# drtconway/zotmer

Hardware: AMD Instinct MI355X
Metric: Gk-mers/sec kmerize k=25 on synthetic 150bp FASTQ; achieved HBM GB/s fraction (higher is better)
Workload: dtype u64

## Files before the change

### zotmer_amd/csrc/strand_blocks.hip

```cpp
#include "tile_group.hpp"

namespace zk {

constexpr int SB_ITEMS = 16, SB_GROUPS = 2048;
constexpr u32 SB_GROUP_MAX = 128;
typedef TileSortSmem<SB_ITEMS, SB_GROUPS, false> StrandSmem;
constexpr int SB_BLOCK_BITS = 18;

__global__ __launch_bounds__(256) void strand_mirror_kernel(const u64* __restrict__ in, const u64* __restrict__ cuts, const u64* __restrict__ incl,
                                                            const u64* __restrict__ nwords, u32 chunks, int pack, int K, u64* __restrict__ out_m,
                                                            MirrorHist mh, const u32* __restrict__ list, u64* cursor, u64 m_cap) {
    __shared__ u32 bins[4 * 512];
    __shared__ u64 placed;
    const bool hist = mh.passes > 0;
    if (hist) {
        for (int q = threadIdx.x; q < 4 * 512; q += blockDim.x) bins[q] = 0;
        __syncthreads();
    }
    const u64 maxc = (1ull << pack) - 1;
    for (u32 t = blockIdx.x; t < chunks; t += gridDim.x) {
        const u32 v = list ? list[t] : t;
        const u64 cnt = nwords[v];
        u64 dst0 = incl[v] - cnt;
        if (list) {
            if (threadIdx.x == 0) placed = atomicAdd(cursor, cnt);
            __syncthreads();
            dst0 = placed;
            __syncthreads();
            if (dst0 + cnt > m_cap) continue;
        }
        const u64* src = in + cuts[v];
        for (u64 i0 = threadIdx.x; i0 < cnt; i0 += 4ull * blockDim.x) {
            u64 w4[4];
#pragma unroll
            for (int q = 0; q < 4; q++) {
                const u64 i = i0 + (u64)q * blockDim.x;
                w4[q] = i < cnt ? src[i] : 0;
            }
#pragma unroll
            for (int q = 0; q < 4; q++) {
                const u64 i = i0 + (u64)q * blockDim.x;
                if (i >= cnt) break;
                const u64 mw = (revcomp(K, w4[q] >> pack) << pack) | (w4[q] & maxc);
                out_m[dst0 + i] = mw;
                if (hist) {
#pragma unroll
                    for (int p = 0; p < 4; p++)
                        if (p < mh.passes) atomicAdd(&bins[p * 512 + ((u32)(mw >> mh.shift[p]) & ((1u << mh.bits[p]) - 1u))], 1u);
                }
            }
        }
    }
    if (hist) {
        __syncthreads();
        for (int q = threadIdx.x; q < mh.passes * 512; q += blockDim.x)
            if (bins[q]) atomicAdd(&mh.raw[q], (u64)bins[q]);
    }
}

__global__ void strand_starts_kernel(const u64* __restrict__ m, u64 n, int shift, u64* __restrict__ start) {
    const u32 g = blockIdx.x * blockDim.x + threadIdx.x;
    if (g > (1u << SB_BLOCK_BITS)) return;
    u64 lo = 0, hi = n;
    if (g == (1u << SB_BLOCK_BITS)) lo = n;
    while (lo < hi) {
        const u64 mid = (lo + hi) >> 1;
        if ((m[mid] >> shift) < (u64)g) lo = mid + 1; else hi = mid;
    }
    start[g] = lo;
}

struct StrandArgs {
    const u64* cw;
    const u64* cuts; const u64* nwords; const u64* incl;
    const u64* m;
    const u64* mstart;
    u64* ok; u32* oc;
    int pack;
    int pshift;
    u32* n_declined;
    u32* declined;
};

__device__ __forceinline__ bool strand_crowded(const StrandSmem& sm, int tid) {
    static_assert(SB_GROUPS == 4 * TS_BLOCK, "four groups a thread");
    u32 big = 0;
#pragma unroll
    for (int q = 0; q < 4; q++) big |= sm.start[4 * tid + q + 1] - sm.start[4 * tid + q] > SB_GROUP_MAX ? 1u : 0u;
    return __syncthreads_or((int)big) != 0;
}

__device__ __forceinline__ void strand_write(const StrandSmem& sm, const TileMap& tm, u32 m, u64* ok, u32* oc, int pack, int tid) {
    const u64 maxc = (1ull << pack) - 1;
    constexpr int E = 2;
    for (u32 i0 = (u32)tid; i0 < m; i0 += E * TS_BLOCK) {
        u32 i[E], place[E];
        u64 mine[E];
#pragma unroll
        for (int e = 0; e < E; e++) i[e] = i0 + e * TS_BLOCK;
        tile_rank<E, false>(sm, tm, i, m, mine, place);
#pragma unroll
        for (int e = 0; e < E; e++) {
            if (i[e] >= m) break;
            ok[place[e]] = mine[e] >> pack;
            oc[place[e]] = (u32)(mine[e] & maxc);
        }
    }
}

__global__ __launch_bounds__(TS_BLOCK, 2 * TS_BLOCK / 256) void strand_block_union_kernel(StrandArgs a) {
    using S = StrandSmem;
    constexpr u32 CAP = S::CAP;
    static_assert(sizeof(S) <= 80 * 1024, "two workgroups per CU");
    __shared__ S sm;
    const u32 b = blockIdx.x;
    const u64 nc = a.nwords[b], m0 = a.mstart[b], nm = a.mstart[b + 1] - m0;
    const u64 n = nc + nm;
    if (n == 0) return;
    if (n > CAP) {
        if (threadIdx.x == 0) a.declined[atomicAdd(a.n_declined, 1u)] = b;
        return;
    }
    int tid = threadIdx.x;
    asm volatile("" : "+v"(tid));
    const u32 m = (u32)n;
    const TileMap tm = tile_group<SB_ITEMS, SB_GROUPS, false>(sm, a.cw, nullptr, a.cuts[b], m, a.pshift, tid, a.m, m0, (u32)nc);
    if (strand_crowded(sm, tid)) {
        if (tid == 0) a.declined[atomicAdd(a.n_declined, 1u)] = b;
        return;
    }
    const u64 out0 = a.incl[b] - nc + m0;
    strand_write(sm, tm, m, a.ok + out0, a.oc + out0, a.pack, tid);
}

constexpr int SB_SPLIT = 256;
struct StrandBigSmem {
    StrandSmem t;
    u64 sp[SB_SPLIT];
    u32 cnt[SB_SPLIT + 2];
    u32 tile[SB_SPLIT + 2];
    u32 ntiles, gcount, fail;
};

__global__ __launch_bounds__(TS_BLOCK) void strand_big_block_kernel(StrandArgs a, u32 n_list, u64* __restrict__ scratch, u32* __restrict__ fail) {
    using S = StrandBigSmem;
    constexpr u32 CAP = StrandSmem::CAP, R = SB_SPLIT + 1;
    __shared__ S sm;
    u64* gat = scratch + (u64)blockIdx.x * CAP;
    const int lane = threadIdx.x & 63;
    for (u32 li = blockIdx.x; li < n_list; li += gridDim.x) {
        int tid = threadIdx.x;
        asm volatile("" : "+v"(tid));
        const u32 b = a.declined[li];
        const u64 nc = a.nwords[b], m0 = a.mstart[b], nm = a.mstart[b + 1] - m0, n = nc + nm;
        const u64* C = a.cw + a.cuts[b];
        const u64* M = a.m + m0;
        auto entry = [&](u64 i) -> u64 { return i < nc ? C[i] : M[i - nc]; };
        const u64 bmin = (u64)b << a.pshift, bmax = bmin | ((1ull << a.pshift) - 1ull);
        const u64 out0 = a.incl[b] - nc + m0;
        u64* cand = sm.t.keys;
        if (tid < SB_SPLIT) cand[tid] = entry((u64)tid * n / SB_SPLIT);
        if (tid == 0) { sm.fail = 0; sm.gcount = 0; }
        if (tid < (int)R + 1) sm.cnt[tid] = 0;
        __syncthreads();
        if (tid < SB_SPLIT) {
            const u64 v = cand[tid];
            u32 r = 0;
            for (int q = 0; q < SB_SPLIT; q++) { const u64 o = cand[q]; r += (o < v || (o == v && q < tid)) ? 1u : 0u; }
            sm.sp[r] = v;
        }
        __syncthreads();
        auto range_of = [&](u64 v) -> u32 {
            u32 lo = 0, hi = SB_SPLIT;
            while (lo < hi) { const u32 mid = (lo + hi) >> 1; if (sm.sp[mid] <= v) lo = mid + 1; else hi = mid; }
            return lo;
        };
        for (u64 i = tid; i < n; i += TS_BLOCK) atomicAdd(&sm.cnt[range_of(entry(i))], 1u);
        __syncthreads();
        if (tid == 0) {
            u32 acc = 0, nt = 0, eb = 0;
            sm.tile[nt++] = 0;
            for (u32 j = 0; j < R; j++) {
                const u32 tot = sm.cnt[j];
                if (tot > CAP) { sm.fail = 1; break; }
                if (acc + tot > CAP) { sm.tile[nt++] = j; acc = 0; }
                acc += tot;
                sm.cnt[j] = eb;
                eb += tot;
            }
            sm.cnt[R] = eb;
            sm.tile[nt] = R;
            sm.ntiles = nt;
        }
        __syncthreads();
        if (sm.fail) {
            if (tid == 0) atomicOr(fail, 1u);
            continue;
        }
        const u32 ntiles = sm.ntiles;
        for (u32 t = 0; t < ntiles; t++) {
            const u32 ra = sm.tile[t], rb = sm.tile[t + 1];
            const u64 vlo = ra == 0 ? bmin : sm.sp[ra - 1];
            const u64 vhi = rb == R ? bmax : sm.sp[rb - 1] - 1;
            const u32 m = sm.cnt[rb] - sm.cnt[ra];
            if (m == 0) continue;
            for (u64 i0 = 0; i0 < n; i0 += TS_BLOCK) {
                const u64 i = i0 + tid;
                const u64 v = i < n ? entry(i) : 0;
                const bool in = i < n && v >= vlo && v <= vhi;
                const u64 bal = __ballot(in);
                u32 base = 0;
                if (lane == 0 && bal) base = atomicAdd(&sm.gcount, (u32)__popcll(bal));
                base = (u32)__shfl((int)base, 0, 64);
                if (in) gat[base + popc_below(bal)] = v;
            }
            __threadfence_block();
            __syncthreads();
            const TileMap tm = tile_group<SB_ITEMS, SB_GROUPS, false>(sm.t, gat, nullptr, 0, m, a.pshift, tid, nullptr, 0, ~0u, true, vlo, vhi);
            if (strand_crowded(sm.t, tid)) {
                if (tid == 0) atomicOr(fail, 1u);
                break;
            }
            const u64 o = out0 + sm.cnt[ra];
            strand_write(sm.t, tm, m, a.ok + o, a.oc + o, a.pack, tid);
            if (tid == 0) sm.gcount = 0;
            __syncthreads();
        }
        __syncthreads();
    }
}

constexpr int DS_ITEMS = 22, DS_GROUPS = 4096;
typedef TileSortSmem<DS_ITEMS, DS_GROUPS, false> BlockSortSmem;
static_assert(BlockSortSmem::CAP == 11264, "a dedupe2_kernel table");

__global__ __launch_bounds__(TS_BLOCK) void dedupe_sort_blocks_kernel(u64* __restrict__ w, const u64* __restrict__ cuts, const u64* __restrict__ nwords,
                                                                     u32 chunks, int pshift) {
    constexpr u32 CAP = BlockSortSmem::CAP;
    __shared__ BlockSortSmem sm;
    for (u32 v = blockIdx.x; v < chunks; v += gridDim.x) {
        const u64 n = nwords[v];
        if (n < 2 || n > CAP) continue;
        int tid = threadIdx.x;
        asm volatile("" : "+v"(tid));
        const u32 m = (u32)n;
        u64* out = w + cuts[v];
        const TileMap tm = tile_group<DS_ITEMS, DS_GROUPS, false>(sm, w, nullptr, cuts[v], m, pshift, tid);
        constexpr int E = 2;
        for (u32 i0 = (u32)tid; i0 < m; i0 += E * TS_BLOCK) {
            u32 i[E], place[E];
            u64 mine[E];
#pragma unroll
            for (int e = 0; e < E; e++) i[e] = i0 + e * TS_BLOCK;
            tile_rank<E, false>(sm, tm, i, m, mine, place);
#pragma unroll
            for (int e = 0; e < E; e++)
                if (i[e] < m) out[place[e]] = mine[e];
        }
        __syncthreads();
    }
}

int dedupe_sort_blocks(zk_ctx* c, DedupeResult& r) {
    if (!r.unsorted || r.n_out == 0) { r.unsorted = false; return ZK_OK; }
    prof_begin(c, ZK_PROF_RLE, 16 * r.n_out);
    hipLaunchKernelGGL(dedupe_sort_blocks_kernel, dim3(r.chunks < (u32)c->num_cus ? r.chunks : (u32)c->num_cus), dim3(TS_BLOCK), 0, c->stream, r.work, r.cuts,
                       r.nwords, r.chunks, r.tag_bits + r.pack);
    prof_end(c);
    ZK_HIP(c, hipGetLastError());
    r.unsorted = false;
    return ZK_OK;
}

int strand_blocks(zk_ctx* c, const DedupeResult& r, u64* keys_buf, uint64_t buf_words, int K, u64* out_k, u32* out_c, uint64_t cap,
                  uint64_t* n_out) {
    *n_out = 0;
    const uint64_t uc = r.n_out;
    if (uc == 0) return ZK_OK;
    if (!(K & 1) || r.n_big || r.chunks != (1u << SB_BLOCK_BITS)) return fail(c, ZK_EINTERNAL, "strand_blocks: K %d, %u big counts, %u blocks", K, r.n_big, r.chunks);
    const uint64_t a8w = ((8 * uc + 255) & ~255ull) / 8;
    if (2 * a8w > buf_words) return fail(c, ZK_EINTERNAL, "strand_blocks: %llu words do not fit twice in %llu", (unsigned long long)uc, (unsigned long long)buf_words);
    if (2 * uc > cap) return fail(c, ZK_ENOSPC, "output holds %llu entries, the table has %llu", (unsigned long long)cap, (unsigned long long)(2 * uc));
    const int pk = r.pack, key_bits = 2 * K + pk, lo_bit = key_bits - SB_BLOCK_BITS;
    u64* mw = keys_buf;
    u64* malt = keys_buf + a8w;
    MirrorHist mh = {};
    bool fused = r.m_emitted && r.m_words >= keys_buf && r.m_words + r.m_cap <= keys_buf + buf_words && uc <= r.m_cap && c->sort_variant == 3;
    if (fused) {
        const PassPlan plan = sort_plan_upper(c, key_bits, lo_bit);
        fused = plan.passes == r.mh.passes;
        for (int p = 0; fused && p < plan.passes; p++) fused = plan.shift[p] == r.mh.shift[p] && plan.bits[p] == r.mh.bits[p];
        const uint64_t before = (uint64_t)(r.m_words - keys_buf), behind = buf_words - before;
        if (before < a8w && behind < 2 * a8w) fused = false;
        if (fused) malt = before >= a8w ? keys_buf : r.m_words + a8w;
    }
    if (fused) {
        mw = r.m_words;
        mh = r.mh;
        uint64_t placed = r.m_placed;
        prof_begin(c, ZK_PROF_SELECT, 16 * uc);
        if (r.n_retry) {
            hipLaunchKernelGGL(strand_mirror_kernel, dim3(grid_cap(c, r.n_retry, 8)), dim3(256), 0, c->stream, r.work, r.cuts, r.incl, r.nwords, r.n_retry, pk, K,
                               mw, mh, r.retry, &c->d_scalars->dedupe_m_cursor, (u64)r.m_cap);
        }
        prof_end(c);
        if (r.n_retry) {
            ZK_HIP(c, hipGetLastError());
            ZK_TRY(fetch(c, &c->h_scalars->dedupe_m_cursor));
            ZK_TRY(stream_sync(c));
            placed = c->h_scalars->dedupe_m_cursor;
        }
        if (placed != uc) return fail(c, ZK_EINTERNAL, "strand_blocks: %llu mirror words for %llu entries", (unsigned long long)placed, (unsigned long long)uc);
    } else {
        if (c->sort_variant == 3) {
            const PassPlan plan = sort_plan_upper(c, key_bits, lo_bit);
            if (plan.passes <= 4) {
                ZK_TRY(arena_alloc(c, sizeof(u64) * MAX_PASSES * 512, (void**)&mh.raw));
                ZK_HIP(c, hipMemsetAsync(mh.raw, 0, sizeof(u64) * MAX_PASSES * 512, c->stream));
                mh.passes = plan.passes;
                for (int p = 0; p < plan.passes; p++) { mh.shift[p] = plan.shift[p]; mh.bits[p] = plan.bits[p]; }
            }
        }
        prof_begin(c, ZK_PROF_SELECT, 16 * uc);
        hipLaunchKernelGGL(strand_mirror_kernel, dim3((u32)c->num_cus * 8), dim3(256), 0, c->stream, r.work, r.cuts, r.incl, r.nwords, r.chunks, pk, K, mw, mh,
                           (const u32*)nullptr, (u64*)nullptr, (u64)0);
        prof_end(c);
        ZK_HIP(c, hipGetLastError());
    }
    u64* sk = nullptr;
    if (mh.passes) ZK_TRY(sort_keys_upper_counted(c, mw, malt, uc, key_bits, lo_bit, mh.raw, &sk));
    else ZK_TRY(sort_keys_upper(c, mw, malt, uc, key_bits, lo_bit, &sk));
    u64* mstart;
    u32* declined;
    ZK_TRY(arena_alloc(c, sizeof(u64) * ((1ull << SB_BLOCK_BITS) + 1), (void**)&mstart));
    ZK_TRY(arena_alloc(c, sizeof(u32) * r.chunks, (void**)&declined));
    StrandArgs a = {};
    a.cw = r.work; a.cuts = r.cuts; a.nwords = r.nwords; a.incl = r.incl; a.m = sk; a.mstart = mstart;
    a.ok = out_k; a.oc = out_c; a.pack = pk; a.pshift = lo_bit;
    a.n_declined = &c->d_scalars->strand.n_declined;
    a.declined = declined;
    u32* fail = &c->d_scalars->strand.fail;
    prof_begin(c, ZK_PROF_UNION, 8 * 2 * uc + 12 * 2 * uc);
    hipLaunchKernelGGL(strand_starts_kernel, dim3(((1u << SB_BLOCK_BITS) + 256) / 256), dim3(256), 0, c->stream, sk, (u64)uc, lo_bit, mstart);
    ZK_HIP(c, hipMemsetAsync(&c->d_scalars->strand, 0, sizeof(zk_strand_counters), c->stream));
    hipLaunchKernelGGL(strand_block_union_kernel, dim3(r.chunks), dim3(TS_BLOCK), 0, c->stream, a);
    prof_end(c);
    ZK_HIP(c, hipGetLastError());
    ZK_TRY(fetch(c, &c->h_scalars->strand));
    ZK_TRY(check_device_error(c));
    const uint32_t n_declined = c->h_scalars->strand.n_declined;
    bool other_way = n_declined && c->strand_blocks == 3;
    if (n_declined && !other_way) {
        const uint32_t grid = n_declined < 2u * (uint32_t)c->num_cus ? n_declined : 2u * (uint32_t)c->num_cus;
        u64* scratch;
        ZK_TRY(arena_alloc(c, sizeof(u64) * StrandSmem::CAP * grid, (void**)&scratch));
        prof_begin(c, ZK_PROF_UNION, 0);
        hipLaunchKernelGGL(strand_big_block_kernel, dim3(grid), dim3(TS_BLOCK), 0, c->stream, a, n_declined, scratch, fail);
        prof_end(c);
        ZK_HIP(c, hipGetLastError());
        ZK_TRY(fetch(c, &c->h_scalars->strand));
        ZK_TRY(check_device_error(c));
        other_way = c->h_scalars->strand.fail != 0;
    }
    if (!other_way) {
        *n_out = 2 * uc;
        return ZK_OK;
    }
    DedupeResult rs = r;
    ZK_TRY(dedupe_sort_blocks(c, rs));
    char* aux;
    ZK_TRY(aux_require(c, 8 * a8w, &aux));
    ZK_TRY(dedupe_finish(c, rs, (u64*)aux, nullptr, nullptr, K, 0, nullptr, nullptr, true));
    u64* ms = nullptr;
    ZK_TRY(sort_keys_upper(c, sk, sk == mw ? malt : mw, uc, key_bits, pk, &ms));
    return union_sum_packed_ab(c, (const u64*)aux, uc, ms, uc, pk, out_k, out_c, cap, n_out, true);
}

}
```

Measured before the change: 169.4.

## Add 32-bit tag path for strand block union when low key bits fit

When the k-mer bits below the block prefix fit in 32 bits (2K-18 <= 32, true for k=25), the block union kernel now stores only 32-bit tags plus separate counts in shared memory instead of full 64-bit packed words. It groups with LDS atomics and a scan, then ranks each element within its group by comparison counting with an unrolled first window, and rebuilds the output key as block index shifted above the tag. This reduces shared-memory footprint and bandwidth and avoids the generic tile_group/tile_rank path. The cost is added template code and a quadratic-in-group-size rank step that relies on groups staying small.

```diff
diff --git a/zotmer_amd/csrc/strand_blocks.hip b/zotmer_amd/csrc/strand_blocks.hip
--- a/zotmer_amd/csrc/strand_blocks.hip
+++ b/zotmer_amd/csrc/strand_blocks.hip
@@ -80,9 +80,12 @@
     int pshift;
     u32* n_declined;
     u32* declined;
+    int below;
+    int gshift;
 };
 
-__device__ __forceinline__ bool strand_crowded(const StrandSmem& sm, int tid) {
+template <class S>
+__device__ __forceinline__ bool strand_crowded(const S& sm, int tid) {
     static_assert(SB_GROUPS == 4 * TS_BLOCK, "four groups a thread");
     u32 big = 0;
 #pragma unroll
@@ -108,8 +111,119 @@
     }
 }
 
+struct StrandTagSmem {
+    static constexpr int CAP = TS_BLOCK * SB_ITEMS;
+    alignas(16) u32 tags[CAP + 16];
+    u32 cnts[CAP];
+    alignas(16) u32 start[SB_GROUPS + 8 + 64];
+    u32 wsum[TS_BLOCK / 64];
+};
+constexpr int SB_RANK_E = 2, SB_RANK_FIRST = 8;
+
+__device__ __forceinline__ void strand_tag_group(StrandTagSmem& sm, const u64* __restrict__ c, const u64* __restrict__ mm, u32 nc, u32 m,
+                                                 int pack, int below, int gshift, int tid) {
+    constexpr int G = SB_GROUPS, NW = TS_BLOCK / 64;
+    static_assert(G == 4 * TS_BLOCK && StrandTagSmem::CAP <= 8192, "four groups a thread in the scan; group | place << 12 in a word");
+    const int lane = tid & 63, wave = __builtin_amdgcn_readfirstlane(tid >> 6);
+    const u32 tmask = below >= 32 ? ~0u : (1u << below) - 1u, cmask = (u32)((1ull << pack) - 1ull);
+    u32 tag[SB_ITEMS], cnt[SB_ITEMS];
+#pragma unroll
+    for (int j = 0; j < SB_ITEMS; j++) {
+        const u32 i = (u32)j * TS_BLOCK + tid, ic = i < m ? i : m - 1;
+        const u64 w = ic < nc ? c[ic] : mm[ic - nc];
+        tag[j] = __builtin_amdgcn_alignbit((u32)(w >> 32), (u32)w, (u32)pack) & tmask;
+        cnt[j] = (u32)w & cmask;
+    }
+    reinterpret_cast<uint4*>(sm.start)[tid] = make_uint4(0, 0, 0, 0);
+    __syncthreads();
+    u32 gp[SB_ITEMS];
+#pragma unroll
+    for (int j = 0; j < SB_ITEMS; j++) {
+        const u32 i = (u32)j * TS_BLOCK + tid;
+        gp[j] = i < m ? tag[j] >> gshift : (u32)(G + 8 + lane);
+    }
+#pragma unroll
+    for (int j = 0; j < SB_ITEMS; j++) gp[j] |= atomicAdd(&sm.start[gp[j]], 1u) << 12;
+    __syncthreads();
+    {
+        uint4* z = reinterpret_cast<uint4*>(sm.start);
+        const uint4 cq = z[tid];
+        const u32 sum = cq.x + cq.y + cq.z + cq.w;
+        const u32 inc = wave_incl_scan_u32(sum);
+        if (lane == 63) sm.wsum[wave] = inc;
+        __syncthreads();
+        u32 run = inc - sum;
+#pragma unroll
+        for (int w = 0; w < NW; w++) run += w < wave ? sm.wsum[w] : 0u;
+        uint4 sq;
+        sq.x = run; run += cq.x; sq.y = run; run += cq.y; sq.z = run; run += cq.z; sq.w = run;
+        z[tid] = sq;
+        if (tid == 0) sm.start[G] = m;
+    }
+    __syncthreads();
+    u32 p[SB_ITEMS];
+#pragma unroll
+    for (int j = 0; j < SB_ITEMS; j++) p[j] = sm.start[gp[j] & 4095u];
+#pragma unroll
+    for (int j = 0; j < SB_ITEMS; j++) {
+        const u32 i = (u32)j * TS_BLOCK + tid;
+        p[j] = i < m ? p[j] + (gp[j] >> 12) : i;
+    }
+#pragma unroll
+    for (int j = 0; j < SB_ITEMS; j++) { sm.tags[p[j]] = tag[j]; sm.cnts[p[j]] = cnt[j]; }
+    __syncthreads();
+}
+
+template <int E>
+__device__ __forceinline__ void strand_tag_write(const StrandTagSmem& sm, u32 m, u64 hi, int gshift, u64* __restrict__ ok, u32* __restrict__ oc, int tid) {
+    constexpr int F = SB_RANK_FIRST;
+    static_assert(F + 3 <= 16, "the padding of StrandTagSmem::tags");
+    auto before = [](u32 to, u32 q, u32 g1, u32 tm, u32 at) -> u32 {
+        return (u32)(q < g1) & ((u32)(to < tm) | ((u32)(to == tm) & (u32)(q < at)));
+    };
+    for (u32 i0 = (u32)tid; i0 < m; i0 += E * TS_BLOCK) {
+        u32 at[E], mine[E], cnt[E], g0[E], g1[E], o[E][F], place[E];
+#pragma unroll
+        for (int e = 0; e < E; e++) {
+            at[e] = i0 + e * TS_BLOCK < m ? i0 + e * TS_BLOCK : 0u;
+            mine[e] = sm.tags[at[e]];
+            cnt[e] = sm.cnts[at[e]];
+        }
+#pragma unroll
+        for (int e = 0; e < E; e++) {
+            const u32 g = mine[e] >> gshift;
+            g0[e] = sm.start[g]; g1[e] = sm.start[g + 1];
+        }
+#pragma unroll
+        for (int e = 0; e < E; e++)
+#pragma unroll
+            for (int r = 0; r < F; r++) o[e][r] = sm.tags[g0[e] + r];
+#pragma unroll
+        for (int e = 0; e < E; e++) {
+            u32 rank = 0;
+#pragma unroll
+            for (int r = 0; r < F; r++) rank += before(o[e][r], g0[e] + r, g1[e], mine[e], at[e]);
+            for (u32 q0 = g0[e] + F; q0 < g1[e]; q0 += 4) {
+                u32 p4[4];
+#pragma unroll
+                for (int r = 0; r < 4; r++) p4[r] = sm.tags[q0 + r];
+#pragma unroll
+                for (int r = 0; r < 4; r++) rank += before(p4[r], q0 + r, g1[e], mine[e], at[e]);
+            }
+            place[e] = g0[e] + rank;
+        }
+#pragma unroll
+        for (int e = 0; e < E; e++) {
+            if (i0 + e * TS_BLOCK >= m) break;
+            ok[place[e]] = hi | mine[e];
+            oc[place[e]] = cnt[e];
+        }
+    }
+}
+
+template <bool TAGS>
 __global__ __launch_bounds__(TS_BLOCK, 2 * TS_BLOCK / 256) void strand_block_union_kernel(StrandArgs a) {
-    using S = StrandSmem;
+    using S = std::conditional_t<TAGS, StrandTagSmem, StrandSmem>;
     constexpr u32 CAP = S::CAP;
     static_assert(sizeof(S) <= 80 * 1024, "two workgroups per CU");
     __shared__ S sm;
@@ -124,13 +238,22 @@
     int tid = threadIdx.x;
     asm volatile("" : "+v"(tid));
     const u32 m = (u32)n;
-    const TileMap tm = tile_group<SB_ITEMS, SB_GROUPS, false>(sm, a.cw, nullptr, a.cuts[b], m, a.pshift, tid, a.m, m0, (u32)nc);
-    if (strand_crowded(sm, tid)) {
-        if (tid == 0) a.declined[atomicAdd(a.n_declined, 1u)] = b;
-        return;
-    }
     const u64 out0 = a.incl[b] - nc + m0;
-    strand_write(sm, tm, m, a.ok + out0, a.oc + out0, a.pack, tid);
+    if constexpr (TAGS) {
+        strand_tag_group(sm, a.cw + a.cuts[b], a.m + m0, (u32)nc, m, a.pack, a.below, a.gshift, tid);
+        if (strand_crowded(sm, tid)) {
+            if (tid == 0) a.declined[atomicAdd(a.n_declined, 1u)] = b;
+            return;
+        }
+        strand_tag_write<SB_RANK_E>(sm, m, (u64)b << a.below, a.gshift, a.ok + out0, a.oc + out0, tid);
+    } else {
+        const TileMap tm = tile_group<SB_ITEMS, SB_GROUPS, false>(sm, a.cw, nullptr, a.cuts[b], m, a.pshift, tid, a.m, m0, (u32)nc);
+        if (strand_crowded(sm, tid)) {
+            if (tid == 0) a.declined[atomicAdd(a.n_declined, 1u)] = b;
+            return;
+        }
+        strand_write(sm, tm, m, a.ok + out0, a.oc + out0, a.pack, tid);
+    }
 }
 
 constexpr int SB_SPLIT = 256;
@@ -337,13 +460,15 @@
     StrandArgs a = {};
     a.cw = r.work; a.cuts = r.cuts; a.nwords = r.nwords; a.incl = r.incl; a.m = sk; a.mstart = mstart;
     a.ok = out_k; a.oc = out_c; a.pack = pk; a.pshift = lo_bit;
+    a.below = 2 * K - SB_BLOCK_BITS; a.gshift = a.below > 11 ? a.below - 11 : 0;
     a.n_declined = &c->d_scalars->strand.n_declined;
     a.declined = declined;
     u32* fail = &c->d_scalars->strand.fail;
     prof_begin(c, ZK_PROF_UNION, 8 * 2 * uc + 12 * 2 * uc);
     hipLaunchKernelGGL(strand_starts_kernel, dim3(((1u << SB_BLOCK_BITS) + 256) / 256), dim3(256), 0, c->stream, sk, (u64)uc, lo_bit, mstart);
     ZK_HIP(c, hipMemsetAsync(&c->d_scalars->strand, 0, sizeof(zk_strand_counters), c->stream));
-    hipLaunchKernelGGL(strand_block_union_kernel, dim3(r.chunks), dim3(TS_BLOCK), 0, c->stream, a);
+    if (a.below <= 32) hipLaunchKernelGGL(strand_block_union_kernel<true>, dim3(r.chunks), dim3(TS_BLOCK), 0, c->stream, a);
+    else hipLaunchKernelGGL(strand_block_union_kernel<false>, dim3(r.chunks), dim3(TS_BLOCK), 0, c->stream, a);
     prof_end(c);
     ZK_HIP(c, hipGetLastError());
     ZK_TRY(fetch(c, &c->h_scalars->strand));
```

Result: faster. 173.5, median of 6 (+2.4%).
